# BadgerTechnologies/navigation

Hardware: AMD Instinct MI355X
Metric: scored trajectories/sec (whole node) + costmap inflation cells/sec, 400x400 map (higher is better)
Workload: dtype f64

## Files before the change

### navigation_amd/csrc/costmap_kernels.hip

```cpp
#include "navgpu_device.h"

namespace navgpu {

__global__ void k_fill_u8(uint8_t* dst, uint8_t v, size_t n) {
  size_t i = (size_t)blockIdx.x * blockDim.x + threadIdx.x;
  size_t stride = (size_t)gridDim.x * blockDim.x;
  uint32_t w = v * 0x01010101u;
  uint4 q = make_uint4(w, w, w, w);
  size_t n16 = n / 16;
  for (size_t k = i; k < n16; k += stride) reinterpret_cast<uint4*>(dst)[k] = q;
  for (size_t k = n16 * 16 + i; k < n; k += stride) dst[k] = v;
}
__global__ void k_fill_u32(uint32_t* dst, uint32_t v, size_t n) {
  size_t i = (size_t)blockIdx.x * blockDim.x + threadIdx.x;
  size_t stride = (size_t)gridDim.x * blockDim.x;
  for (size_t k = i; k < n; k += stride) dst[k] = v;
}
void launch_fill_u8(uint8_t* dst, uint8_t v, size_t n, hipStream_t s) {
  if (!n) return;
  size_t blocks = (n / 16 + 255) / 256;
  if (blocks < 1) blocks = 1;
  if (blocks > 4096) blocks = 4096;
  hipLaunchKernelGGL(k_fill_u8, dim3((unsigned)blocks), dim3(256), 0, s, dst, v, n);
}
void launch_fill_u32(uint32_t* dst, uint32_t v, size_t n, hipStream_t s) {
  if (!n) return;
  size_t blocks = (n + 255) / 256;
  if (blocks > 4096) blocks = 4096;
  hipLaunchKernelGGL(k_fill_u32, dim3((unsigned)blocks), dim3(256), 0, s, dst, v, n);
}

__global__ void k_static_interpret(uint8_t* dst, const int8_t* occ, uint32_t cells, uint32_t cells_padded, uint32_t count,
                                   int track_unknown_space, int trinary, int lethal_threshold, int unknown_cost_value) {
  uint32_t i = blockIdx.x * blockDim.x + threadIdx.x;
  if (i >= cells) return;
  uint8_t value = (uint8_t)occ[i];
  uint8_t lethal_thr = (uint8_t)lethal_threshold;
  uint8_t unknown = (uint8_t)unknown_cost_value;
  uint8_t out;
  if (track_unknown_space && value == unknown)
    out = kNoInfo;
  else if (!track_unknown_space && value == unknown)
    out = kFree;
  else if (value >= lethal_thr)
    out = kLethal;
  else if (trinary)
    out = kFree;
  else {
    double scale = (double)value / lethal_thr;
    out = (uint8_t)(scale * kLethal);
  }
  for (uint32_t k = 0; k < count; ++k) dst[(size_t)k * cells_padded + i] = out;
}
void launch_static_interpret(uint8_t* dst, const int8_t* occ, uint32_t cells, uint32_t cells_padded, uint32_t count,
                             int track_unknown_space, int trinary, int lethal_threshold, int unknown_cost_value, hipStream_t s) {
  hipLaunchKernelGGL(k_static_interpret, dim3((cells + 255) / 256), dim3(256), 0, s, dst, occ, cells, cells_padded, count,
                     track_unknown_space, trinary, lethal_threshold, unknown_cost_value);
}

__global__ void k_export_window(const uint8_t* master, uint32_t nx, uint32_t x0, uint32_t y0, uint32_t w, uint32_t h, int8_t* out) {
  const uint32_t i = blockIdx.x * blockDim.x + threadIdx.x;
  if (i >= w * h) return;
  const uint32_t y = i / w, x = i - y * w;
  const uint32_t v = master[(size_t)(y0 + y) * nx + x0 + x];
  int8_t o;
  if (v == 0) o = 0;
  else if (v == 253) o = 99;
  else if (v == 254) o = 100;
  else if (v == 255) o = -1;
  else o = (int8_t)(1 + (97 * ((int)v - 1)) / 251);
  out[i] = o;
}
void launch_export_window(const uint8_t* master, uint32_t nx, uint32_t x0, uint32_t y0, uint32_t w, uint32_t h, int8_t* out, hipStream_t s) {
  hipLaunchKernelGGL(k_export_window, dim3((w * h + 255) / 256), dim3(256), 0, s, master, nx, x0, y0, w, h, out);
}

template <class T>
__global__ __launch_bounds__(256) void k_shift(const T* src, T* dst, CostmapDev cm, uint32_t first, T fill) {
  const uint32_t inst = first + blockIdx.y;
  const int ox = cm.shift[2 * inst], oy = cm.shift[2 * inst + 1];
  const T* s = src + (size_t)inst * cm.cells_padded;
  T* d = dst + (size_t)inst * cm.cells_padded;
  for (uint32_t i = blockIdx.x * blockDim.x + threadIdx.x; i < cm.cells; i += gridDim.x * blockDim.x) {
    const int y = i / cm.nx, x = i - y * cm.nx;
    const int sx = x + ox, sy = y + oy;
    d[i] = (sx >= 0 && sy >= 0 && sx < (int)cm.nx && sy < (int)cm.ny) ? s[sy * cm.nx + sx] : fill;
  }
}
void launch_shift_u8(const uint8_t* src, uint8_t* dst, const CostmapDev& cm, uint32_t first, uint32_t count, uint8_t fill, hipStream_t s) {
  dim3 grid(min((cm.cells + 255) / 256, 64u), count);
  hipLaunchKernelGGL(k_shift<uint8_t>, grid, dim3(256), 0, s, src, dst, cm, first, fill);
}
void launch_shift_u32(const uint32_t* src, uint32_t* dst, const CostmapDev& cm, uint32_t first, uint32_t count, uint32_t fill, hipStream_t s) {
  dim3 grid(min((cm.cells + 255) / 256, 64u), count);
  hipLaunchKernelGGL(k_shift<uint32_t>, grid, dim3(256), 0, s, src, dst, cm, first, fill);
}

template <class F>
__device__ __forceinline__ void raytrace3d(uint32_t nx, double x0, double y0, double z0, double x1, double y1, double z1,
                                           uint32_t max_length, F&& at) {
  int dx = int(x1) - int(x0), dy = int(y1) - int(y0), dz = int(z1) - int(z0);
  uint32_t abs_dx = dx < 0 ? -dx : dx, abs_dy = dy < 0 ? -dy : dy, abs_dz = dz < 0 ? -dz : dz;
  int offset_dx = dx > 0 ? 1 : -1;
  int offset_dy = (dy > 0 ? 1 : -1) * (int)nx;
  int offset_dz = dz > 0 ? 1 : -1;
  uint32_t z_mask = ((1u << 16) | 1u) << (uint32_t)z0;
  uint32_t offset = (uint32_t)y0 * nx + (uint32_t)x0;
  double dist = sqrt((x0 - x1) * (x0 - x1) + (y0 - y1) * (y0 - y1) + (z0 - z1) * (z0 - z1));
  double scale = fmin(1.0, (double)max_length / dist);
  uint32_t abs_da, abs_db, abs_dc;
  int off_a, off_b, off_c, role_a, role_b, role_c;
  uint32_t mmax = abs_dy > abs_dz ? abs_dy : abs_dz;
  if (abs_dx >= mmax) {
    abs_da = abs_dx; abs_db = abs_dy; abs_dc = abs_dz;
    off_a = offset_dx; off_b = offset_dy; off_c = offset_dz;
    role_a = 0; role_b = 0; role_c = 1;
  } else if (abs_dy >= abs_dz) {
    abs_da = abs_dy; abs_db = abs_dx; abs_dc = abs_dz;
    off_a = offset_dy; off_b = offset_dx; off_c = offset_dz;
    role_a = 0; role_b = 0; role_c = 1;
  } else {
    abs_da = abs_dz; abs_db = abs_dx; abs_dc = abs_dy;
    off_a = offset_dz; off_b = offset_dx; off_c = offset_dy;
    role_a = 1; role_b = 0; role_c = 0;
  }
  auto step = [&](int role, int v) {
    if (role == 0)
      offset += v;
    else {
      if (v > 0)
        z_mask <<= 1;
      else
        z_mask >>= 1;
    }
  };
  uint32_t lim = (uint32_t)(scale * abs_da);
  uint32_t end = lim < abs_da ? lim : abs_da;
  int error_b = abs_da / 2, error_c = abs_da / 2;
  for (uint32_t i = 0; i < end; ++i) {
    at(offset, z_mask);
    step(role_a, off_a);
    error_b += abs_db;
    error_c += abs_dc;
    if ((uint32_t)error_b >= abs_da) {
      step(role_b, off_b);
      error_b -= abs_da;
    }
    if ((uint32_t)error_c >= abs_da) {
      step(role_c, off_c);
      error_c -= abs_da;
    }
  }
  at(offset, z_mask);
// ... 275 lines not shown
  b.store(st->bounds);
  int x0, xn, y0, yn;
  enforceBounds(g, b.min_x, b.min_y, x0, y0);
  enforceBounds(g, b.max_x, b.max_y, xn, yn);
  x0 = x0 > 0 ? x0 : 0;
  xn = ((int)g.nx < xn + 1) ? (int)g.nx : xn + 1;
  y0 = y0 > 0 ? y0 : 0;
  yn = ((int)g.ny < yn + 1) ? (int)g.ny : yn + 1;
  st->box[0] = x0;
  st->box[1] = xn;
  st->box[2] = y0;
  st->box[3] = yn;
  st->box_valid = !(xn < x0 || yn < y0);
  return st->box_valid;
}

__device__ __forceinline__ void clearFootprintPolygon(const CostmapDev& cm, const Geom& g, uint32_t inst, uint8_t* layer, uint32_t tid,
                                                      uint32_t* s_vx, uint32_t* s_vy, uint32_t* colmin, uint32_t* colmax, int* s_poly_ok) {
  const uint32_t nfp = cm.fp_n[inst];
  if (tid == 0) *s_poly_ok = nfp >= 3;
  __syncthreads();
  if (tid < nfp) {
    uint32_t mx, my;
    bool ok = worldToMap(g, cm.fp_world[((size_t)inst * kMaxFootprint + tid) * 2], cm.fp_world[((size_t)inst * kMaxFootprint + tid) * 2 + 1], mx, my);
    s_vx[tid] = mx;
    s_vy[tid] = my;
    if (!ok) atomicAnd(s_poly_ok, 0);
  }
  __syncthreads();
  if (!*s_poly_ok) return;
  uint32_t minx = 0xFFFFFFFFu, maxx = 0;
  for (uint32_t i = 0; i < nfp; ++i) {
    minx = s_vx[i] < minx ? s_vx[i] : minx;
    maxx = s_vx[i] > maxx ? s_vx[i] : maxx;
  }
  const uint32_t span = maxx - minx + 1;
  if (span > 1024) return;
  for (uint32_t c = tid; c < span; c += blockDim.x) {
    colmin[c] = 0xFFFFFFFFu;
    colmax[c] = 0;
  }
  __syncthreads();
  if (tid < nfp) {
    uint32_t e1 = (tid + 1 == nfp) ? 0 : tid + 1;
    raytrace2d(g.nx, s_vx[tid], s_vy[tid], s_vx[e1], s_vy[e1], 0xFFFFFFFFu, [&](uint32_t off) {
      uint32_t y = off / g.nx, x = off - y * g.nx;
      atomicMin(&colmin[x - minx], y);
      atomicMax(&colmax[x - minx], y);
    });
  }
  __syncthreads();
  for (uint32_t c = tid >> 4; c < span; c += blockDim.x >> 4) {
    uint32_t lo = colmin[c], hi = colmax[c];
    if (lo == 0xFFFFFFFFu) continue;
    for (uint32_t y = lo + (tid & 15); y <= hi; y += 16) layer[y * g.nx + minx + c] = kFree;
  }
}

template <bool VOXEL>
__global__ __launch_bounds__(256) void k_obstacle(CostmapDev cm, uint32_t first, const double* bounds_io_in, double* bounds_io_out,
                                                  int only_bounds) {
  const uint32_t inst = first + blockIdx.x, tid = threadIdx.x;
  ObstacleGrids L;
  L.g = Geom{cm.origin[2 * inst], cm.origin[2 * inst + 1], cm.res, cm.nx, cm.ny};
  L.layer = cm.obst + (size_t)inst * cm.cells_padded;
  L.vox = VOXEL ? cm.voxel + (size_t)inst * cm.cells_padded : nullptr;
  L.size_z = VOXEL ? (uint32_t)(cm.z_voxels > 16 ? 16 : cm.z_voxels) : 0;
  L.unknown_thr = VOXEL ? (uint32_t)(cm.unknown_threshold + (16 - cm.z_voxels)) : 0;
  L.mark_thr = VOXEL ? (uint32_t)cm.mark_threshold : 0;
  InstCostmapState* st = cm.state + inst;
  __shared__ double red[4][4];
  __shared__ int s_box_valid;
  __shared__ uint32_t colmin[1024], colmax[1024];
  __shared__ uint32_t s_vx[kMaxFootprint], s_vy[kMaxFootprint];
  __shared__ int s_poly_ok;

  const bool has_obs_layer = (cm.layers & (NAVGPU_LAYER_OBSTACLE | NAVGPU_LAYER_VOXEL)) && cm.obs_enabled;
  BoundsAcc b{1e30, 1e30, -1e30, -1e30};
  if (tid == 0) boundsSeed(cm, L.g, st, bounds_io_in, only_bounds, has_obs_layer, b);

  if (has_obs_layer) {
    const uint32_t ob = inst * cm.max_obs, oe = ob + cm.obs_count[inst];
    const float* inst_points = cm.points + (size_t)inst * cm.max_points * 3;
    for (int pass = 0; pass < (VOXEL ? 2 : 1); ++pass) {
      for (uint32_t o = ob; o < oe; ++o) {
        const ObsCsr obs = cm.obs[o];
        if (!(obs.flags & NAVGPU_OBS_CLEARING)) continue;
        if (!VOXEL)
          clearRays2D(L, obs, inst_points + (size_t)obs.first_point * 3, tid, b);
        else
          clearRaysVoxel(cm, L, obs, inst_points + (size_t)obs.first_point * 3, pass, tid, b);
      }
      __syncthreads();
    }
    if (VOXEL && L.mark_thr > 0)
      markPointsOrdered(cm, L, ob, oe, inst_points, cm.mark_seq + (size_t)inst * cm.max_points, tid, b);
    else
      for (uint32_t o = ob; o < oe; ++o) {
        const ObsCsr obs = cm.obs[o];
        if (!(obs.flags & NAVGPU_OBS_MARKING)) continue;
        markPoints<VOXEL>(cm, L, obs, inst_points + (size_t)obs.first_point * 3, tid, b);
      }
    footprintTouch(cm, inst, tid, b);
  }

  reduceBounds(b, red, tid);
  if (tid == 0) s_box_valid = finishBounds(cm, L.g, st, b, bounds_io_out, only_bounds);
  __syncthreads();
  if (has_obs_layer && cm.footprint_clearing && s_box_valid)
    clearFootprintPolygon(cm, L.g, inst, L.layer, tid, s_vx, s_vy, colmin, colmax, &s_poly_ok);
}

__global__ __launch_bounds__(256) void k_reset_bounding_box(CostmapDev cm, uint32_t first, const double* boxes_world) {
  const uint32_t inst = first + blockIdx.x;
  const Geom g{cm.origin[2 * inst], cm.origin[2 * inst + 1], cm.res, cm.nx, cm.ny};
  const double* bw = boxes_world + 4 * blockIdx.x;
  int x0, y0, xn, yn;
  enforceBounds(g, bw[0], bw[1], x0, y0);
  enforceBounds(g, bw[2], bw[3], xn, yn);
  uint8_t* layer = cm.obst + (size_t)inst * cm.cells_padded;
  if (xn > x0 && yn > y0) {
    const uint32_t w = (uint32_t)(xn - x0), n = w * (uint32_t)(yn - y0);
    for (uint32_t i = threadIdx.x; i < n; i += blockDim.x) layer[(uint32_t)(y0 + i / w) * g.nx + (uint32_t)x0 + i % w] = cm.obstacle_default;
  }
  if (threadIdx.x == 0) {
    InstCostmapState* st = cm.state + inst;
    if (!st->has_extra_bounds) {
      st->extra[0] = st->extra[1] = 1e6;
      st->extra[2] = st->extra[3] = -1e6;
    }
    st->extra[0] = (bw[0] < st->extra[0]) ? bw[0] : st->extra[0];
    st->extra[1] = (bw[1] < st->extra[1]) ? bw[1] : st->extra[1];
    st->extra[2] = (st->extra[2] < bw[2]) ? bw[2] : st->extra[2];
    st->extra[3] = (st->extra[3] < bw[3]) ? bw[3] : st->extra[3];
    st->has_extra_bounds = 1;
  }
}
__global__ __launch_bounds__(256) void k_reset_window(uint8_t* grid, size_t stride, uint32_t nx, uint32_t x0, uint32_t y0, uint32_t xn, uint32_t yn, uint8_t value) {
  uint8_t* gp = grid + (size_t)blockIdx.x * stride;
  const uint32_t w = xn - x0, n = w * (yn - y0);
  for (uint32_t i = threadIdx.x; i < n; i += blockDim.x) gp[(y0 + i / w) * nx + x0 + i % w] = value;
}
void launch_reset_window(uint8_t* grid, size_t stride, uint32_t count, uint32_t nx, uint32_t x0, uint32_t y0, uint32_t xn, uint32_t yn, uint8_t value, hipStream_t s) {
  hipLaunchKernelGGL(k_reset_window, dim3(count), dim3(256), 0, s, grid, stride, nx, x0, y0, xn, yn, value);
}
void launch_reset_bounding_box(const CostmapDev& cm, uint32_t first, uint32_t count, const double* boxes_world, hipStream_t s) {
  hipLaunchKernelGGL(k_reset_bounding_box, dim3(count), dim3(256), 0, s, cm, first, boxes_world);
}

struct UpdateBox {
  int x0, y0, xn, yn;
};
__device__ __forceinline__ bool updateBox(const CostmapDev& cm, const int32_t* boxes, uint32_t k, uint32_t inst, UpdateBox& box) {
  if (boxes) {
    box = UpdateBox{boxes[4 * k + 0], boxes[4 * k + 1], boxes[4 * k + 2], boxes[4 * k + 3]};
    return true;
  }
  const InstCostmapState* st = cm.state + inst;
  if (!st->box_valid) return false;
  box.x0 = st->box[0];
  box.xn = st->box[1];
  box.y0 = st->box[2];
  box.yn = st->box[3];
  return true;
}
__device__ __forceinline__ UpdateBox inflateBox(const UpdateBox& box, int R, uint32_t nx, uint32_t ny) {
  return UpdateBox{max(0, box.x0 - R), max(0, box.y0 - R), min((int)nx, box.xn + R), min((int)ny, box.yn + R)};
}

void launch_obstacle(const CostmapDev& cm, uint32_t first, uint32_t count, const double* bounds_in, int only_bounds, hipStream_t s) {
  double* bounds_out = const_cast<double*>(bounds_in);
  if (cm.layers & NAVGPU_LAYER_VOXEL)
    hipLaunchKernelGGL(k_obstacle<true>, dim3(count), dim3(256), 0, s, cm, first, bounds_in, bounds_out, only_bounds);
  else
    hipLaunchKernelGGL(k_obstacle<false>, dim3(count), dim3(256), 0, s, cm, first, bounds_in, bounds_out, only_bounds);
}

__global__ __launch_bounds__(256) void k_merge(CostmapDev cm, uint32_t first, const int32_t* boxes, int static_received, int layer_only) {
  const uint32_t inst = first + blockIdx.y;
  UpdateBox box;
  if (!updateBox(cm, boxes, blockIdx.y, inst, box)) return;
  const int x0 = box.x0, y0 = box.y0, xn = box.xn, yn = box.yn;
  const uint32_t q = blockIdx.x * blockDim.x + threadIdx.x;
  const uint32_t base = q * 16;
  if (base >= cm.cells) return;
  const int row_first = base / cm.nx, row_last = (min(base + 15, cm.cells - 1)) / cm.nx;
  if (row_last < y0 || row_first >= yn) return;
  bool inside = false;
  if (row_first == row_last) {
    const int gx = base - row_first * cm.nx;
    if (gx + 15 < x0 || gx >= xn) return;
    inside = gx >= x0 && gx + 15 < xn && base + 15 < cm.cells && !layer_only;
  }
  const size_t off = (size_t)inst * cm.cells_padded + base;
  uint4 mv = make_uint4(0, 0, 0, 0);
  if (!inside) mv = *reinterpret_cast<const uint4*>(cm.master + off);
  const bool has_static = (cm.layers & NAVGPU_LAYER_STATIC) && static_received && !layer_only && !cm.stat_roll && cm.stat;
  const bool roll_static = cm.stat_roll != nullptr && !layer_only;
  double tfm[8] = {1, 0, 0, 0, 0, 1, 0, 0};
  double m_ox = 0, m_oy = 0;
  if (roll_static) {
    const double* T = cm.stat_tf + (size_t)inst * 12;
    tfm[0] = T[0]; tfm[1] = T[1]; tfm[2] = T[2]; tfm[3] = T[9];
    tfm[4] = T[3]; tfm[5] = T[4]; tfm[6] = T[5]; tfm[7] = T[10];
    m_ox = cm.origin[2 * inst];
    m_oy = cm.origin[2 * inst + 1];
  }
  const bool has_obst = (cm.layers & (NAVGPU_LAYER_OBSTACLE | NAVGPU_LAYER_VOXEL)) && cm.obs_enabled;
  uint4 sv = has_static ? *reinterpret_cast<const uint4*>(cm.stat + off) : make_uint4(0, 0, 0, 0);
  uint4 lv = has_obst ? *reinterpret_cast<const uint4*>(cm.obst + off) : make_uint4(0, 0, 0, 0);
  uint32_t mw[4] = {mv.x, mv.y, mv.z, mv.w}, sw[4] = {sv.x, sv.y, sv.z, sv.w}, lw[4] = {lv.x, lv.y, lv.z, lv.w};
  int y = row_first;
  int x = base - row_first * cm.nx;
  bool changed = false;
#pragma unroll
  for (int k = 0; k < 16; ++k) {
    if (base + k < cm.cells && x >= x0 && x < xn && y >= y0 && y < yn) {
      const int sh = (k & 3) * 8;
      uint8_t m = layer_only ? (uint8_t)((mw[k >> 2] >> sh) & 0xFF) : cm.master_default;
      if (has_static) {
        uint8_t sc = (sw[k >> 2] >> sh) & 0xFF;
        if (!cm.static_use_maximum)
          m = sc;
        else if (sc != kNoInfo && (m == kNoInfo || m < sc))
          m = sc;
      }
      if (roll_static) {
        const double wx = m_ox + (x + 0.5) * cm.res, wy = m_oy + (y + 0.5) * cm.res;
        const double px = tfm[0] * wx + tfm[1] * wy + tfm[2] * 0.0 + tfm[3];
        const double py = tfm[4] * wx + tfm[5] * wy + tfm[6] * 0.0 + tfm[7];
        if (!(px < cm.stat_ox || py < cm.stat_oy)) {
          const uint32_t smx = (uint32_t)(int)((px - cm.stat_ox) / cm.stat_res), smy = (uint32_t)(int)((py - cm.stat_oy) / cm.stat_res);
          if (smx < cm.stat_nx && smy < cm.stat_ny) {
            const uint8_t sc = cm.stat_roll[(size_t)smy * cm.stat_nx + smx];
            m = cm.static_use_maximum ? (sc > m ? sc : m) : sc;
          }
        }
      }
      if (has_obst) {
        uint8_t lc = (lw[k >> 2] >> sh) & 0xFF;
        if (lc != kNoInfo) {
          if (cm.combination_method == 0)
            m = lc;
          else if (cm.combination_method == 1 && (m == kNoInfo || m < lc))
            m = lc;
        }
      }
      mw[k >> 2] = (mw[k >> 2] & ~(0xFFu << sh)) | ((uint32_t)m << sh);
      changed = true;
    }
    if (++x == (int)cm.nx) {
      x = 0;
      ++y;
    }
  }
  if (changed) *reinterpret_cast<uint4*>(cm.master + off) = make_uint4(mw[0], mw[1], mw[2], mw[3]);
}

void launch_merge(const CostmapDev& cm, uint32_t first, uint32_t count, const int32_t* boxes, hipStream_t s, bool layer_only) {
  uint32_t groups = (cm.cells + 15) / 16;
  dim3 grid((groups + 255) / 256, count);
  hipLaunchKernelGGL(k_merge, grid, dim3(256), 0, s, cm, first, boxes, cm.static_received, layer_only ? 1 : 0);
}

constexpr int kTile = 64;
__global__ __launch_bounds__(256) void k_inflate(CostmapDev cm, uint32_t first, const int32_t* boxes) {
  extern __shared__ __align__(16) uint8_t lds[];
  const uint32_t inst = first + blockIdx.z;
  const int R = (int)cm.R;
  UpdateBox box;
  if (!updateBox(cm, boxes, blockIdx.z, inst, box)) return;
  box = inflateBox(box, R, cm.nx, cm.ny);
  const int min_i = box.x0, min_j = box.y0, max_i = box.xn, max_j = box.yn;
  const int tx0 = blockIdx.x * kTile, ty0 = blockIdx.y * kTile;
  if (tx0 - R >= max_i || tx0 + kTile + R <= min_i || ty0 - R >= max_j || ty0 + kTile + R <= min_j) return;

  const int W = kTile + 2 * R;
  const int WS = (W + 3) & ~3;
  uint8_t* seed = lds;
  uint8_t* hd = seed + W * WS;
  uint8_t* lut = hd + W * kTile;
  __shared__ int s_any;
  const uint32_t tid = threadIdx.x;
  uint8_t* master = cm.master + (size_t)inst * cm.cells_padded;
  if (tid == 0) s_any = 0;
  for (int i = tid; i < (R + 2) * (R + 2); i += blockDim.x) lut[i] = cm.lut[i];
  __syncthreads();
  int any = 0;
  for (int i = tid; i < W * W; i += blockDim.x) {
    int ly = i / W, lx = i - ly * W;
    int gx = tx0 - R + lx, gy = ty0 - R + ly;
    uint8_t f = 0;
    if (gx >= min_i && gx < max_i && gy >= min_j && gy < max_j) f = master[gy * cm.nx + gx] == kLethal;
    seed[ly * WS + lx] = f;
    any |= f;
  }
  if (any) s_any = 1;
  __syncthreads();
  if (!s_any) return;
  for (int i = tid; i < W * kTile; i += blockDim.x) {
    int ly = i / kTile, c = i - ly * kTile;
    const uint8_t* row = seed + ly * WS + c + R;
    uint8_t best = 255;
    for (int d = 0; d <= R; ++d) {
      if (row[d] | row[-d]) {
        best = (uint8_t)d;
        break;
      }
    }
    hd[i] = best;
  }
  __syncthreads();
  const int n = R + 2;
  for (int i = tid; i < kTile * kTile; i += blockDim.x) {
    int ry = i / kTile, c = i - ry * kTile;
    int gx = tx0 + c, gy = ty0 + ry;
    if (gx >= (int)cm.nx || gy >= (int)cm.ny) continue;
    uint8_t cost = 0;
    for (int dy = -R; dy <= R; ++dy) {
      uint8_t h = hd[(ry + R + dy) * kTile + c];
      if (h != 255) {
        int ady = dy < 0 ? -dy : dy;
        uint8_t cc = lut[h * n + ady];
        cost = cc > cost ? cc : cost;
      }
    }
    if (cost == 0) continue;
    uint8_t old = master[gy * cm.nx + gx];
    uint8_t nv = (old == kNoInfo && cost >= kInscribed) ? cost : (old > cost ? old : cost);
    if (nv != old) master[gy * cm.nx + gx] = nv;
  }
}

constexpr int kBX = 64, kBY = 32;
template <int RT>
__global__ __launch_bounds__(256) void k_inflate_bits(CostmapDev cm, uint32_t first, uint32_t count, const int32_t* boxes) {
  const uint32_t tbx = blockIdx.x >> 3, tby = blockIdx.y, rz = blockIdx.z * 8u + (blockIdx.x & 7u);
  if (rz >= count) return;
  const uint32_t inst = first + rz;
  const int R = RT > 0 ? RT : (int)cm.R;
  UpdateBox box;
  if (!updateBox(cm, boxes, rz, inst, box)) return;
  box = inflateBox(box, R, cm.nx, cm.ny);
  const int min_i = box.x0, min_j = box.y0, max_i = box.xn, max_j = box.yn;
  const int tx0 = (int)tbx * kBX, ty0 = (int)tby * kBY;
  if (tx0 - R >= max_i || tx0 + kBX + R <= min_i || ty0 - R >= max_j || ty0 + kBY + R <= min_j) return;

  constexpr int kMaxHR = kBY + 2 * 14;
  constexpr int kOct = (kMaxHR + 7) / 8;
  __shared__ uint32_t s_rows[kMaxHR][4];
  __shared__ uint32_t s_hd[kOct + 1][kBX];
  __shared__ uint8_t s_lut2[256];
  __shared__ int s_any;
  __shared__ uint32_t s_rowany[2];
  const uint32_t tid = threadIdx.x, lane = tid & 63, wave = tid >> 6;
  const int HR = kBY + 2 * R;
  uint8_t* master = cm.master + (size_t)inst * cm.cells_padded;
  if (tid == 0) s_any = 0;
  if (tid < 2) s_rowany[tid] = 0;
  s_lut2[tid] = cm.lut2[tid];
  __syncthreads();
  int any = 0;
  uint32_t rows_lo = 0, rows_hi = 0;
  constexpr int kSeedIt = (kMaxHR + 3) / 4;
  uint8_t cell[kSeedIt][2];
  const int gxa = tx0 - 32 + (int)lane, gxb = gxa + 64;
  const int lo_x = max(min_i, tx0 - R), lo_y = max(min_j, ty0 - R);
  const int hi_x = max(lo_x, min(max_i, tx0 + kBX + R) - 1), hi_y = max(lo_y, min(max_j, ty0 + kBY + R) - 1);
  const int cxa = min(min(max(gxa, lo_x), hi_x), (int)cm.nx - 1), cxb = min(min(max(gxb, lo_x), hi_x), (int)cm.nx - 1);
  const bool xa_ok = gxa >= min_i && gxa < max_i && gxa >= tx0 - R && gxa < tx0 + kBX + R;
  const bool xb_ok = gxb >= min_i && gxb < max_i && gxb >= tx0 - R && gxb < tx0 + kBX + R;
#pragma unroll
  for (int it = 0; it < kSeedIt; ++it) {
    const int gy = ty0 - R + (int)wave + 4 * it;
    const int cy = min(min(max(gy, lo_y), hi_y), (int)cm.ny - 1);
    cell[it][0] = master[cy * cm.nx + cxa];
    cell[it][1] = master[cy * cm.nx + cxb];
  }
#pragma unroll
  for (int it = 0; it < kSeedIt; ++it) {
    const int r = (int)wave + 4 * it, gy = ty0 - R + r;
    if (r < HR) {
      const bool row_ok = gy >= min_j && gy < max_j;
#pragma unroll
      for (int half = 0; half < 2; ++half) {
        const unsigned long long m = __ballot(row_ok && (half ? xb_ok : xa_ok) && cell[it][half] == kLethal);
        if (lane == 0) {
          s_rows[r][2 * half] = (uint32_t)m;
          s_rows[r][2 * half + 1] = (uint32_t)(m >> 32);
        }
        any |= m != 0ull;
        if (m != 0ull) {
          if (r < 32)
            rows_lo |= 1u << r;
          else
            rows_hi |= 1u << (r - 32);
        }
      }
    }
  }
  if (any && lane == 0) {
    s_any = 1;
    if (rows_lo) atomicOr(&s_rowany[0], rows_lo);
    if (rows_hi) atomicOr(&s_rowany[1], rows_hi);
  }
  __syncthreads();
  if (!s_any) return;
  const uint32_t lowmask = (1u << R) - 1u;
  for (int o = wave; o * 8 < HR; o += 4) {
    uint32_t packed = 0;
#pragma unroll
    for (int k = 0; k < 8; ++k) {
      const int r = o * 8 + k;
      uint32_t h = 15;
      if (r < HR && (s_rows[r][0] | s_rows[r][1] | s_rows[r][2] | s_rows[r][3]) != 0u) {
        const uint32_t sft = 32u + lane - (uint32_t)R;
        const uint32_t wi = sft >> 5, bs = sft & 31u;
        const unsigned long long two = ((unsigned long long)s_rows[r][wi + 1 < 4 ? wi + 1 : 3] << 32) | s_rows[r][wi];
        const uint32_t q = (uint32_t)(two >> bs);
        const uint32_t qr = q >> R;
        const uint32_t ql = q & lowmask;
        uint32_t dr = 15, dl = 15;
        if (qr & ((2u << R) - 1u)) dr = (uint32_t)__builtin_ctz(qr & ((2u << R) - 1u));
        if (ql) dl = (uint32_t)R - (31u - (uint32_t)__builtin_clz(ql));
        h = dr < dl ? dr : dl;
      }
      packed |= h << (4 * k);
    }
    s_hd[o][lane] = packed;
  }
  __syncthreads();
  uint32_t hw[5];
#pragma unroll
  for (int k = 0; k < 5; ++k) hw[k] = (wave + k) * 8 < (uint32_t)HR ? s_hd[wave + k][lane] : 0xFFFFFFFFu;
  if (__ballot((hw[0] & hw[1] & hw[2] & hw[3] & hw[4]) != 0xFFFFFFFFu) == 0ull) return;
  const int gx = tx0 + (int)lane;
  const int R2 = R * R;
  uint32_t bestr[8] = {0xFFFFu, 0xFFFFu, 0xFFFFu, 0xFFFFu, 0xFFFFu, 0xFFFFu, 0xFFFFu, 0xFFFFu};
  if (RT > 0) {
    const unsigned long long rowany = (((unsigned long long)s_rowany[1] << 32) | s_rowany[0]) >> (8u * wave);
    const uint32_t ra_lo = __builtin_amdgcn_readfirstlane((uint32_t)rowany), ra_hi = __builtin_amdgcn_readfirstlane((uint32_t)(rowany >> 32));
#pragma unroll
    for (int p = 0; p < 8 + 2 * RT; ++p) {
      if (((p < 32 ? ra_lo >> (p & 31) : ra_hi >> (p & 31)) & 1u) != 0u) {
        const uint32_t h = (hw[p >> 3] >> (4 * (p & 7))) & 15u;
        const uint32_t hh = h * h;
#pragma unroll
        for (int j = 0; j < 8; ++j) {
          const int dy = p - RT - j;
          if (dy >= -RT && dy <= RT) {
            const uint32_t d2 = hh + (uint32_t)(dy * dy);
            bestr[j] = d2 < bestr[j] ? d2 : bestr[j];
          }
        }
      }
    }
  }
#pragma unroll
  for (int j = 0; j < 8; ++j) {
    const int gy = ty0 + (int)wave * 8 + j;
    uint32_t best = bestr[j];
    if (RT == 0) {
      for (int dy = -R; dy <= R; ++dy) {
        const int p = j + R + dy;
        const uint32_t wsel = p >> 3;
        const uint32_t word = wsel == 0 ? hw[0] : (wsel == 1 ? hw[1] : (wsel == 2 ? hw[2] : (wsel == 3 ? hw[3] : hw[4])));
        const uint32_t h = (word >> (4 * (p & 7))) & 15u;
        const uint32_t d2 = h * h + (uint32_t)(dy * dy);
        best = d2 < best ? d2 : best;
      }
    }
    if (best > (uint32_t)R2 || gx >= (int)cm.nx || gy >= (int)cm.ny) continue;
    const uint8_t cost = s_lut2[best];
    if (cost == 0) continue;
    const uint8_t old = master[gy * cm.nx + gx];
    const uint8_t nv = (old == kNoInfo && cost >= kInscribed) ? cost : (old > cost ? old : cost);
    if (nv != old) master[gy * cm.nx + gx] = nv;
  }
}

constexpr uint32_t kPqSeenWords = 5120, kPqWinBytes = 65536;
constexpr size_t kPqLdsBytes = 150 * 1024;
constexpr uint32_t kPqTabEntries = 66 * 66;
__global__ __launch_bounds__(64) void k_inflate_pq(CostmapDev cm, uint32_t first, const int32_t* boxes) {
  extern __shared__ __align__(16) uint8_t pq_sm[];
  const uint32_t inst = first + blockIdx.x;
  const uint32_t tid = threadIdx.x;
  UpdateBox box;
  if (!updateBox(cm, boxes, blockIdx.x, inst, box)) return;
  uint8_t* master = cm.master + (size_t)inst * cm.cells_padded;
  uint8_t* seen_g = cm.pq_seen + (size_t)inst * cm.cells_padded;
  PqCell* heap_g = cm.pq_heap + (size_t)inst * cm.pq_cap;
  const uint32_t size_x = cm.nx, size_y = cm.ny;
  const int R = (int)cm.R;
  const uint32_t n = cm.R + 2;
  box = inflateBox(box, R, size_x, size_y);
  const int min_i = box.x0, min_j = box.y0, max_i = box.xn, max_j = box.yn;
  if (max_i <= min_i || max_j <= min_j) return;
  const int wx0 = max(0, min_i - R - 1), wy0 = max(0, min_j - R - 1), wx1 = min((int)size_x, max_i + R + 1), wy1 = min((int)size_y, max_j + R + 1);
  const uint32_t ww = (uint32_t)(wx1 - wx0), wh = (uint32_t)(wy1 - wy0), wcells = ww * wh;
  const bool seen_lds = wcells <= kPqSeenWords * 32u, win_lds = wcells <= kPqWinBytes;
  uint16_t* rank = reinterpret_cast<uint16_t*>(pq_sm);
  uint8_t* lut_l = pq_sm + kPqTabEntries * 2;
  const uint32_t seen_off = (kPqTabEntries * 3 + 15u) & ~15u;
  uint32_t* seen_l = reinterpret_cast<uint32_t*>(pq_sm + seen_off);
  const uint32_t win_off = seen_off + (seen_lds ? (((wcells + 31) / 32 * 4 + 15u) & ~15u) : 0u);
  uint8_t* win_l = pq_sm + win_off;
  const uint32_t heap_off = win_off + (win_lds ? ((wcells + 15u) & ~15u) : 0u);
  PqCell* heap_l = reinterpret_cast<PqCell*>(pq_sm + heap_off);
  const long heap_lds = (long)((kPqLdsBytes - heap_off) / sizeof(PqCell));
  for (uint32_t i = tid; i < n * n; i += 64) {
    rank[i] = reinterpret_cast<const uint16_t*>(cm.dist_lut)[i];
    lut_l[i] = cm.lut[i];
  }
  if (seen_lds) {
    for (uint32_t i = tid; i < (wcells + 31) / 32; i += 64) seen_l[i] = 0;
  } else {
    for (uint32_t i = tid * 16; i < cm.cells_padded; i += 64 * 16) *reinterpret_cast<uint4*>(seen_g + i) = make_uint4(0, 0, 0, 0);
  }
  if (win_lds)
    for (uint32_t i = tid; i < wcells; i += 64) {
      const uint32_t y = i / ww, x = i - y * ww;
      win_l[i] = master[(uint32_t)(wy0 + (int)y) * size_x + (uint32_t)(wx0 + (int)x)];
    }
  __syncthreads();
  if (tid == 0) {
    long len = 0;
    auto hget = [&](long i) -> PqCell { return i < heap_lds ? heap_l[i] : heap_g[i]; };
    auto hset = [&](long i, const PqCell& v) {
      if (i < heap_lds)
        heap_l[i] = v;
      else
        heap_g[i] = v;
    };
    auto widx = [&](uint32_t mx, uint32_t my) { return (my - (uint32_t)wy0) * ww + (mx - (uint32_t)wx0); };
    auto seenGet = [&](uint32_t index, uint32_t mx, uint32_t my) -> bool {
      if (seen_lds) {
        const uint32_t w = widx(mx, my);
        return (seen_l[w >> 5] >> (w & 31)) & 1u;
      }
      return seen_g[index] != 0;
    };
    auto seenSet = [&](uint32_t index, uint32_t mx, uint32_t my) {
      if (seen_lds) {
        const uint32_t w = widx(mx, my);
        seen_l[w >> 5] |= 1u << (w & 31);
      } else {
        seen_g[index] = 1;
      }
    };
    auto pushHeap = [&](long hole, const PqCell& value) {
      long parent = (hole - 1) / 2;
      while (hole > 0) {
        const PqCell pv = hget(parent);
        if (!(pv.rank > value.rank)) break;
        hset(hole, pv);
        hole = parent;
        parent = (hole - 1) / 2;
      }
      hset(hole, value);
    };
    auto probe = [&](bool in_map, uint32_t index, uint32_t mx, uint32_t my, uint32_t sx, uint32_t sy) -> uint32_t {
      if (!in_map) return 0xFFFFu;
      const uint32_t dx = mx > sx ? mx - sx : sx - mx, dy = my > sy ? my - sy : sy - my;
      const uint32_t r = rank[dx * n + dy];
      return seenGet(index, mx, my) ? 0xFFFFu : r;
    };
    auto push = [&](uint32_t r, uint32_t index, uint32_t mx, uint32_t my, uint32_t sx, uint32_t sy) {
      if (r == 0xFFFFu) return;
      if ((uint64_t)len >= cm.pq_cap) return;
      PqCell c;
      c.index = index;
      c.rank = (uint16_t)r;
      c.sdx = (int8_t)((int)sx - (int)mx);
      c.sdy = (int8_t)((int)sy - (int)my);
      pushHeap(len++, c);
    };
    auto enqueue = [&](uint32_t index, uint32_t mx, uint32_t my, uint32_t sx, uint32_t sy) { push(probe(true, index, mx, my, sx, sy), index, mx, my, sx, sy); };
    for (int j = min_j; j < max_j; j++)
      for (int i = min_i; i < max_i; i++) {
        const uint32_t index = (uint32_t)j * size_x + (uint32_t)i;
        const uint8_t c0 = win_lds ? win_l[widx((uint32_t)i, (uint32_t)j)] : master[index];
        if (c0 == kLethal) enqueue(index, i, j, i, j);
      }
    while (len > 0) {
      const PqCell cur = hget(0);
      if (len > 1) {
        const PqCell value = hget(len - 1);
        const long l = len - 1;
        long hole = 0, child = 0;
        while (child < (l - 1) / 2) {
          child = 2 * (child + 1);
          const PqCell a = hget(child), b = hget(child - 1);
          if (a.rank > b.rank) {
            child--;
            hset(hole, b);
          } else {
            hset(hole, a);
          }
          hole = child;
        }
        if ((l & 1) == 0 && child == (l - 2) / 2) {
          child = 2 * (child + 1);
          hset(hole, hget(child - 1));
          hole = child - 1;
        }
        pushHeap(hole, value);
      }
      --len;
      const uint32_t index = cur.index;
      const uint32_t my = index / size_x, mx = index - my * size_x;
      if (seenGet(index, mx, my)) continue;
      seenSet(index, mx, my);
      const uint32_t sx = (uint32_t)((int)mx + cur.sdx), sy = (uint32_t)((int)my + cur.sdy);
      const uint32_t dx = mx > sx ? mx - sx : sx - mx, dy = my > sy ? my - sy : sy - my;
      const uint8_t cost = lut_l[dx * n + dy];
      uint8_t* cellp = win_lds ? &win_l[widx(mx, my)] : &master[index];
      const uint8_t old_cost = *cellp;
      if (old_cost == kNoInfo && cost >= kInscribed)
        *cellp = cost;
      else
        *cellp = old_cost > cost ? old_cost : cost;
      const uint32_t r0 = probe(mx > 0, index - 1, mx - 1, my, sx, sy), r1 = probe(my > 0, index - size_x, mx, my - 1, sx, sy),
                     r2 = probe(mx < size_x - 1, index + 1, mx + 1, my, sx, sy), r3 = probe(my < size_y - 1, index + size_x, mx, my + 1, sx, sy);
      push(r0, index - 1, mx - 1, my, sx, sy);
      push(r1, index - size_x, mx, my - 1, sx, sy);
      push(r2, index + 1, mx + 1, my, sx, sy);
      push(r3, index + size_x, mx, my + 1, sx, sy);
    }
  }
  __syncthreads();
  if (win_lds)
    for (uint32_t i = tid; i < wcells; i += 64) {
      const uint32_t y = i / ww, x = i - y * ww;
      master[(uint32_t)(wy0 + (int)y) * size_x + (uint32_t)(wx0 + (int)x)] = win_l[i];
    }
}

void launch_inflate(const CostmapDev& cm, uint32_t first, uint32_t count, const int32_t* boxes, hipStream_t s) {
  if (!cm.infl_enabled) return;
  const int R = (int)cm.R;
  if (cm.infl_pq) {
    if (!cm.pq_heap || !cm.pq_seen || !cm.dist_lut) return;
    hipFuncSetAttribute((const void*)k_inflate_pq, hipFuncAttributeMaxDynamicSharedMemorySize, (int)kPqLdsBytes);
    hipLaunchKernelGGL(k_inflate_pq, dim3(count), dim3(64), kPqLdsBytes, s, cm, first, boxes);
    return;
  }
  if (cm.lut2_ok && R >= 1 && R <= 14) {
    dim3 grid(8u * ((cm.nx + kBX - 1) / kBX), (cm.ny + kBY - 1) / kBY, (count + 7u) / 8u);
    if (R == 11)
      hipLaunchKernelGGL(k_inflate_bits<11>, grid, dim3(256), 0, s, cm, first, count, boxes);
    else
      hipLaunchKernelGGL(k_inflate_bits<0>, grid, dim3(256), 0, s, cm, first, count, boxes);
    return;
  }
  const int W = kTile + 2 * R, WS = (W + 3) & ~3;
  size_t lds = (size_t)W * WS + (size_t)W * kTile + (size_t)(R + 2) * (R + 2);
  dim3 grid((cm.nx + kTile - 1) / kTile, (cm.ny + kTile - 1) / kTile, count);
  hipLaunchKernelGGL(k_inflate, grid, dim3(256), lds, s, cm, first, boxes);
}

}
```

Baseline: 6.370 billion.

## Vectorize costmap merge with SWAR word rules and streamline bit-inflation kernel

Result: faster. 6.606 billion (median of 6 runs) (+3.7%).

```diff
diff --git a/navigation_amd/csrc/costmap_kernels.hip b/navigation_amd/csrc/costmap_kernels.hip
--- a/navigation_amd/csrc/costmap_kernels.hip
+++ b/navigation_amd/csrc/costmap_kernels.hip
@@ -1,4 +1,5 @@
 #include "navgpu_device.h"
+#include "costmap_word_rules.h"
 
 namespace navgpu {
 
@@ -580,17 +581,14 @@
   int x0, y0, xn, yn;
 };
 __device__ __forceinline__ bool updateBox(const CostmapDev& cm, const int32_t* boxes, uint32_t k, uint32_t inst, UpdateBox& box) {
-  if (boxes) {
-    box = UpdateBox{boxes[4 * k + 0], boxes[4 * k + 1], boxes[4 * k + 2], boxes[4 * k + 3]};
-    return true;
-  }
   const InstCostmapState* st = cm.state + inst;
-  if (!st->box_valid) return false;
-  box.x0 = st->box[0];
-  box.xn = st->box[1];
-  box.y0 = st->box[2];
-  box.yn = st->box[3];
-  return true;
+  const int32_t* p = boxes ? boxes + 4 * (size_t)k : st->box;
+  const int b0 = p[0], b1 = p[1], b2 = p[2], b3 = p[3];
+  box.x0 = b0;
+  box.y0 = boxes ? b1 : b2;
+  box.xn = boxes ? b2 : b1;
+  box.yn = b3;
+  return boxes ? true : st->box_valid != 0;
 }
 __device__ __forceinline__ UpdateBox inflateBox(const UpdateBox& box, int R, uint32_t nx, uint32_t ny) {
   return UpdateBox{max(0, box.x0 - R), max(0, box.y0 - R), min((int)nx, box.xn + R), min((int)ny, box.yn + R)};
@@ -604,7 +602,53 @@
     hipLaunchKernelGGL(k_obstacle<false>, dim3(count), dim3(256), 0, s, cm, first, bounds_in, bounds_out, only_bounds);
 }
 
-__global__ __launch_bounds__(256) void k_merge(CostmapDev cm, uint32_t first, const int32_t* boxes, int static_received, int layer_only) {
+template <bool ALIGNED, int STATIC, int OBST, bool LAYER_ONLY>
+__global__ __launch_bounds__(256) void k_merge(CostmapDev cm, uint32_t first, const int32_t* boxes, word_rules::FastDiv div_nx,
+                                                     word_rules::FastDiv div_gpr) {
+  using namespace word_rules;
+  const uint32_t inst = first + blockIdx.y;
+  UpdateBox box;
+  if (!updateBox(cm, boxes, blockIdx.y, inst, box)) return;
+  const int x0 = box.x0, y0 = box.y0, xn = box.xn, yn = box.yn;
+  const uint32_t wq = blockIdx.x * 256u + (__builtin_amdgcn_readfirstlane(threadIdx.x) & ~63u);
+  if (wq * 16u >= cm.cells) return;
+  const int wrow_first = (int)fastDiv(wq * 16u, div_nx), wrow_last = (int)fastDiv(min(wq * 16u + 1023u, cm.cells - 1u), div_nx);
+  if (wrow_last < y0 || wrow_first >= yn) return;
+  const uint32_t q = blockIdx.x * 256u + threadIdx.x;
+  const uint32_t base = q * 16u;
+  if (base >= cm.cells) return;
+  uint32_t bits;
+  if (ALIGNED) {
+    const uint32_t gpr = cm.nx >> 4, row = fastDiv(q, div_gpr);
+    bits = ((int)row >= y0 && (int)row < yn) ? boxBits((int)((q - row * gpr) << 4), x0, xn) : 0u;
+  } else {
+    int y = (int)fastDiv(base, div_nx);
+    int x = (int)(base - (uint32_t)y * cm.nx);
+    bits = 0;
+#pragma unroll
+    for (int k = 0; k < 16; ++k) {
+      if (base + k < cm.cells && x >= x0 && x < xn && y >= y0 && y < yn) bits |= 1u << k;
+      if (++x == (int)cm.nx) {
+        x = 0;
+        ++y;
+      }
+    }
+  }
+  if (bits == 0u) return;
+  const size_t off = (size_t)inst * cm.cells_padded + base;
+  const uint4 sv = STATIC ? *reinterpret_cast<const uint4*>(cm.stat + off) : make_uint4(0, 0, 0, 0);
+  const uint4 lv = OBST ? *reinterpret_cast<const uint4*>(cm.obst + off) : make_uint4(0, 0, 0, 0);
+  uint4 mv = make_uint4(0, 0, 0, 0);
+  if (LAYER_ONLY || bits != 0xFFFFu) mv = *reinterpret_cast<const uint4*>(cm.master + off);
+  uint4 out;
+  out.x = mergeWord<STATIC, OBST, LAYER_ONLY>(mv.x, sv.x, lv.x, boxBytes(bits, 0), cm.master_default);
+  out.y = mergeWord<STATIC, OBST, LAYER_ONLY>(mv.y, sv.y, lv.y, boxBytes(bits, 1), cm.master_default);
+  out.z = mergeWord<STATIC, OBST, LAYER_ONLY>(mv.z, sv.z, lv.z, boxBytes(bits, 2), cm.master_default);
+  out.w = mergeWord<STATIC, OBST, LAYER_ONLY>(mv.w, sv.w, lv.w, boxBytes(bits, 3), cm.master_default);
+  *reinterpret_cast<uint4*>(cm.master + off) = out;
+}
+
+__global__ __launch_bounds__(256) void k_merge_bytes(CostmapDev cm, uint32_t first, const int32_t* boxes, int static_received, int layer_only) {
   const uint32_t inst = first + blockIdx.y;
   UpdateBox box;
   if (!updateBox(cm, boxes, blockIdx.y, inst, box)) return;
@@ -685,10 +729,51 @@
   if (changed) *reinterpret_cast<uint4*>(cm.master + off) = make_uint4(mw[0], mw[1], mw[2], mw[3]);
 }
 
+template <bool ALIGNED, int STATIC, int OBST, bool LAYER_ONLY>
+static void launchMergeWords(const CostmapDev& cm, uint32_t first, const int32_t* boxes, dim3 grid, hipStream_t s) {
+  hipLaunchKernelGGL((k_merge<ALIGNED, STATIC, OBST, LAYER_ONLY>), grid, dim3(256), 0, s, cm, first, boxes, word_rules::fastDivOf(cm.nx),
+                     word_rules::fastDivOf(cm.nx >= 16 ? cm.nx >> 4 : 1));
+}
+template <bool ALIGNED, int STATIC>
+static void launchMergeObst(const CostmapDev& cm, uint32_t first, const int32_t* boxes, dim3 grid, hipStream_t s, int obst, bool layer_only) {
+  if (layer_only) {
+    if (STATIC != 0) return;
+    switch (obst) {
+      case 0: return launchMergeWords<ALIGNED, 0, 0, true>(cm, first, boxes, grid, s);
+      case 1: return launchMergeWords<ALIGNED, 0, 1, true>(cm, first, boxes, grid, s);
+      default: return launchMergeWords<ALIGNED, 0, 2, true>(cm, first, boxes, grid, s);
+    }
+  }
+  switch (obst) {
+    case 0: return launchMergeWords<ALIGNED, STATIC, 0, false>(cm, first, boxes, grid, s);
+    case 1: return launchMergeWords<ALIGNED, STATIC, 1, false>(cm, first, boxes, grid, s);
+    default: return launchMergeWords<ALIGNED, STATIC, 2, false>(cm, first, boxes, grid, s);
+  }
+}
+template <bool ALIGNED>
+static void launchMergeStatic(const CostmapDev& cm, uint32_t first, const int32_t* boxes, dim3 grid, hipStream_t s, int stat, int obst, bool layer_only) {
+  switch (stat) {
+    case 0: return launchMergeObst<ALIGNED, 0>(cm, first, boxes, grid, s, obst, layer_only);
+    case 1: return launchMergeObst<ALIGNED, 1>(cm, first, boxes, grid, s, obst, layer_only);
+    default: return launchMergeObst<ALIGNED, 2>(cm, first, boxes, grid, s, obst, layer_only);
+  }
+}
+
 void launch_merge(const CostmapDev& cm, uint32_t first, uint32_t count, const int32_t* boxes, hipStream_t s, bool layer_only) {
   uint32_t groups = (cm.cells + 15) / 16;
   dim3 grid((groups + 255) / 256, count);
-  hipLaunchKernelGGL(k_merge, grid, dim3(256), 0, s, cm, first, boxes, cm.static_received, layer_only ? 1 : 0);
+  if ((cm.stat_roll != nullptr && !layer_only) || cm.cells >= 0x80000000u) {
+    hipLaunchKernelGGL(k_merge_bytes, grid, dim3(256), 0, s, cm, first, boxes, cm.static_received, layer_only ? 1 : 0);
+    return;
+  }
+  const bool has_static = (cm.layers & NAVGPU_LAYER_STATIC) && cm.static_received && !layer_only && cm.stat;
+  const bool has_obst = (cm.layers & (NAVGPU_LAYER_OBSTACLE | NAVGPU_LAYER_VOXEL)) && cm.obs_enabled;
+  const int stat = !has_static ? 0 : (cm.static_use_maximum ? 2 : 1);
+  const int obst = !has_obst ? 0 : (cm.combination_method == 0 ? 1 : (cm.combination_method == 1 ? 2 : 0));
+  if (cm.nx % 16 == 0)
+    launchMergeStatic<true>(cm, first, boxes, grid, s, stat, obst, layer_only);
+  else
+    launchMergeStatic<false>(cm, first, boxes, grid, s, stat, obst, layer_only);
 }
 
 constexpr int kTile = 64;
@@ -761,43 +846,42 @@
 }
 
 constexpr int kBX = 64, kBY = 32;
-template <int RT>
+template <int RT, bool BOXES>
 __global__ __launch_bounds__(256) void k_inflate_bits(CostmapDev cm, uint32_t first, uint32_t count, const int32_t* boxes) {
   const uint32_t tbx = blockIdx.x >> 3, tby = blockIdx.y, rz = blockIdx.z * 8u + (blockIdx.x & 7u);
   if (rz >= count) return;
   const uint32_t inst = first + rz;
   const int R = RT > 0 ? RT : (int)cm.R;
   UpdateBox box;
-  if (!updateBox(cm, boxes, rz, inst, box)) return;
+  if (BOXES) {
+    box = UpdateBox{boxes[4 * rz + 0], boxes[4 * rz + 1], boxes[4 * rz + 2], boxes[4 * rz + 3]};
+  } else {
+    const InstCostmapState* st = cm.state + inst;
+    box = UpdateBox{st->box[0], st->box[2], st->box[1], st->box[3]};
+    if (!st->box_valid) return;
+  }
+  const int tx0 = (int)tbx * kBX, ty0 = (int)tby * kBY;
+  if (tx0 - 2 * R >= box.xn || tx0 + kBX + 2 * R <= box.x0 || ty0 - 2 * R >= box.yn || ty0 + kBY + 2 * R <= box.y0) return;
   box = inflateBox(box, R, cm.nx, cm.ny);
   const int min_i = box.x0, min_j = box.y0, max_i = box.xn, max_j = box.yn;
-  const int tx0 = (int)tbx * kBX, ty0 = (int)tby * kBY;
-  if (tx0 - R >= max_i || tx0 + kBX + R <= min_i || ty0 - R >= max_j || ty0 + kBY + R <= min_j) return;
 
   constexpr int kMaxHR = kBY + 2 * 14;
   constexpr int kOct = (kMaxHR + 7) / 8;
-  __shared__ uint32_t s_rows[kMaxHR][4];
+  __shared__ __align__(16) uint32_t s_rows[kMaxHR][4];
   __shared__ uint32_t s_hd[kOct + 1][kBX];
   __shared__ uint8_t s_lut2[256];
-  __shared__ int s_any;
-  __shared__ uint32_t s_rowany[2];
-  const uint32_t tid = threadIdx.x, lane = tid & 63, wave = tid >> 6;
+  const uint32_t tid = threadIdx.x, lane = tid & 63, wave = (__builtin_amdgcn_readfirstlane(tid) >> 6) & 3u;
   const int HR = kBY + 2 * R;
   uint8_t* master = cm.master + (size_t)inst * cm.cells_padded;
-  if (tid == 0) s_any = 0;
-  if (tid < 2) s_rowany[tid] = 0;
   s_lut2[tid] = cm.lut2[tid];
-  __syncthreads();
-  int any = 0;
-  uint32_t rows_lo = 0, rows_hi = 0;
-  constexpr int kSeedIt = (kMaxHR + 3) / 4;
+  constexpr int kSeedIt = ((RT > 0 ? kBY + 2 * RT : kMaxHR) + 3) / 4;
   uint8_t cell[kSeedIt][2];
   const int gxa = tx0 - 32 + (int)lane, gxb = gxa + 64;
   const int lo_x = max(min_i, tx0 - R), lo_y = max(min_j, ty0 - R);
   const int hi_x = max(lo_x, min(max_i, tx0 + kBX + R) - 1), hi_y = max(lo_y, min(max_j, ty0 + kBY + R) - 1);
   const int cxa = min(min(max(gxa, lo_x), hi_x), (int)cm.nx - 1), cxb = min(min(max(gxb, lo_x), hi_x), (int)cm.nx - 1);
-  const bool xa_ok = gxa >= min_i && gxa < max_i && gxa >= tx0 - R && gxa < tx0 + kBX + R;
-  const bool xb_ok = gxb >= min_i && gxb < max_i && gxb >= tx0 - R && gxb < tx0 + kBX + R;
+  const unsigned long long xa_ok = __builtin_amdgcn_ballot_w64(gxa >= min_i && gxa < max_i && gxa >= tx0 - R && gxa < tx0 + kBX + R);
+  const unsigned long long xb_ok = __builtin_amdgcn_ballot_w64(gxb >= min_i && gxb < max_i && gxb >= tx0 - R && gxb < tx0 + kBX + R);
 #pragma unroll
   for (int it = 0; it < kSeedIt; ++it) {
     const int gy = ty0 - R + (int)wave + 4 * it;
@@ -807,55 +891,45 @@
   }
 #pragma unroll
   for (int it = 0; it < kSeedIt; ++it) {
-    const int r = (int)wave + 4 * it, gy = ty0 - R + r;
+    const int r = (int)wave + 4 * it;
     if (r < HR) {
-      const bool row_ok = gy >= min_j && gy < max_j;
+      const unsigned long long ma = __builtin_amdgcn_ballot_w64(cell[it][0] == kLethal) & xa_ok;
+      const unsigned long long mb = __builtin_amdgcn_ballot_w64(cell[it][1] == kLethal) & xb_ok;
+      *reinterpret_cast<uint4*>(s_rows[r]) = make_uint4((uint32_t)ma, (uint32_t)(ma >> 32), (uint32_t)mb, (uint32_t)(mb >> 32));
+    }
+  }
+  __syncthreads();
+  unsigned long long rowany_tile;
+  {
+    const uint4 w = *reinterpret_cast<const uint4*>(s_rows[lane < (uint32_t)HR ? lane : 0u]);
+    const int gyl = ty0 - R + (int)lane;
+    rowany_tile = __builtin_amdgcn_ballot_w64(lane < (uint32_t)HR && gyl >= min_j && gyl < max_j && (w.x | w.y | w.z | w.w) != 0u);
+  }
+  if (rowany_tile == 0ull) return;
+  const uint32_t lowmask = (1u << R) - 1u;
+  const uint32_t sft = 32u + lane - (uint32_t)R;
+  const uint32_t wi = sft >> 5, bs = sft & 31u;
+  for (int o = wave; o * 8 < HR; o += 4) {
+    const uint32_t oct = (uint32_t)(rowany_tile >> (8 * o)) & 0xFFu;
+    uint32_t near = 0;
+    if (oct != 0u) {
 #pragma unroll
-      for (int half = 0; half < 2; ++half) {
-        const unsigned long long m = __ballot(row_ok && (half ? xb_ok : xa_ok) && cell[it][half] == kLethal);
-        if (lane == 0) {
-          s_rows[r][2 * half] = (uint32_t)m;
-          s_rows[r][2 * half + 1] = (uint32_t)(m >> 32);
+      for (int k = 0; k < 8; ++k) {
+        if ((oct >> k) & 1u) {
+          const int r = o * 8 + k;
+          const unsigned long long two = ((unsigned long long)s_rows[r][wi + 1] << 32) | s_rows[r][wi];
+          const uint32_t q = (uint32_t)(two >> bs);
+          const uint32_t qr = q >> R;
+          const uint32_t ql = q & lowmask;
+          uint32_t dr = 15, dl = 15;
+          if (qr & ((2u << R) - 1u)) dr = (uint32_t)__builtin_ctz(qr & ((2u << R) - 1u));
+          if (ql) dl = (uint32_t)R - (31u - (uint32_t)__builtin_clz(ql));
+          const uint32_t h = dr < dl ? dr : dl;
+          near |= (15u - h) << (4 * k);
         }
-        any |= m != 0ull;
-        if (m != 0ull) {
-          if (r < 32)
-            rows_lo |= 1u << r;
-          else
-            rows_hi |= 1u << (r - 32);
-        }
-      }
-    }
-  }
-  if (any && lane == 0) {
-    s_any = 1;
-    if (rows_lo) atomicOr(&s_rowany[0], rows_lo);
-    if (rows_hi) atomicOr(&s_rowany[1], rows_hi);
-  }
-  __syncthreads();
-  if (!s_any) return;
-  const uint32_t lowmask = (1u << R) - 1u;
-  for (int o = wave; o * 8 < HR; o += 4) {
-    uint32_t packed = 0;
-#pragma unroll
-    for (int k = 0; k < 8; ++k) {
-      const int r = o * 8 + k;
-      uint32_t h = 15;
-      if (r < HR && (s_rows[r][0] | s_rows[r][1] | s_rows[r][2] | s_rows[r][3]) != 0u) {
-        const uint32_t sft = 32u + lane - (uint32_t)R;
-        const uint32_t wi = sft >> 5, bs = sft & 31u;
-        const unsigned long long two = ((unsigned long long)s_rows[r][wi + 1 < 4 ? wi + 1 : 3] << 32) | s_rows[r][wi];
-        const uint32_t q = (uint32_t)(two >> bs);
-        const uint32_t qr = q >> R;
-        const uint32_t ql = q & lowmask;
-        uint32_t dr = 15, dl = 15;
-        if (qr & ((2u << R) - 1u)) dr = (uint32_t)__builtin_ctz(qr & ((2u << R) - 1u));
-        if (ql) dl = (uint32_t)R - (31u - (uint32_t)__builtin_clz(ql));
-        h = dr < dl ? dr : dl;
-      }
-      packed |= h << (4 * k);
-    }
-    s_hd[o][lane] = packed;
+      }
+    }
+    s_hd[o][lane] = ~near;
   }
   __syncthreads();
   uint32_t hw[5];
@@ -864,26 +938,38 @@
   if (__ballot((hw[0] & hw[1] & hw[2] & hw[3] & hw[4]) != 0xFFFFFFFFu) == 0ull) return;
   const int gx = tx0 + (int)lane;
   const int R2 = R * R;
-  uint32_t bestr[8] = {0xFFFFu, 0xFFFFu, 0xFFFFu, 0xFFFFu, 0xFFFFu, 0xFFFFu, 0xFFFFu, 0xFFFFu};
+  uint8_t oldb[8];
+  {
+    const int cgx = min(gx, (int)cm.nx - 1);
+#pragma unroll
+    for (int j = 0; j < 8; ++j) oldb[j] = master[min(ty0 + (int)wave * 8 + j, (int)cm.ny - 1) * cm.nx + cgx];
+  }
+  typedef unsigned short u16x2 __attribute__((ext_vector_type(2)));
+  constexpr unsigned short kFar = 0x7000;
+  u16x2 bestp[4] = {{0xFFFFu, 0xFFFFu}, {0xFFFFu, 0xFFFFu}, {0xFFFFu, 0xFFFFu}, {0xFFFFu, 0xFFFFu}};
   if (RT > 0) {
-    const unsigned long long rowany = (((unsigned long long)s_rowany[1] << 32) | s_rowany[0]) >> (8u * wave);
-    const uint32_t ra_lo = __builtin_amdgcn_readfirstlane((uint32_t)rowany), ra_hi = __builtin_amdgcn_readfirstlane((uint32_t)(rowany >> 32));
+    const unsigned long long rowany = rowany_tile >> (8u * wave);
+    const uint32_t ra_lo = (uint32_t)rowany, ra_hi = (uint32_t)(rowany >> 32);
 #pragma unroll
     for (int p = 0; p < 8 + 2 * RT; ++p) {
       if (((p < 32 ? ra_lo >> (p & 31) : ra_hi >> (p & 31)) & 1u) != 0u) {
         const uint32_t h = (hw[p >> 3] >> (4 * (p & 7))) & 15u;
-        const uint32_t hh = h * h;
+        const uint32_t hh2 = (h * 0x10001u) * h;
 #pragma unroll
-        for (int j = 0; j < 8; ++j) {
-          const int dy = p - RT - j;
-          if (dy >= -RT && dy <= RT) {
-            const uint32_t d2 = hh + (uint32_t)(dy * dy);
-            bestr[j] = d2 < bestr[j] ? d2 : bestr[j];
+        for (int i = 0; i < 4; ++i) {
+          const int dy0 = p - RT - 2 * i, dy1 = dy0 - 1;
+          const bool in0 = dy0 >= -RT && dy0 <= RT, in1 = dy1 >= -RT && dy1 <= RT;
+          if (in0 || in1) {
+            const uint32_t dd = (in0 ? (uint32_t)(dy0 * dy0) : kFar) | ((in1 ? (uint32_t)(dy1 * dy1) : kFar) << 16);
+            bestp[i] = __builtin_elementwise_min(bestp[i], __builtin_bit_cast(u16x2, hh2 + dd));
           }
         }
       }
     }
   }
+  uint32_t bestr[8];
+#pragma unroll
+  for (int j = 0; j < 8; ++j) bestr[j] = (j & 1) ? bestp[j >> 1].y : bestp[j >> 1].x;
 #pragma unroll
   for (int j = 0; j < 8; ++j) {
     const int gy = ty0 + (int)wave * 8 + j;
@@ -898,12 +984,11 @@
         best = d2 < best ? d2 : best;
       }
     }
-    if (best > (uint32_t)R2 || gx >= (int)cm.nx || gy >= (int)cm.ny) continue;
-    const uint8_t cost = s_lut2[best];
-    if (cost == 0) continue;
-    const uint8_t old = master[gy * cm.nx + gx];
+    const uint8_t cost = s_lut2[best < 255u ? best : 255u];
+    const uint8_t old = oldb[j];
     const uint8_t nv = (old == kNoInfo && cost >= kInscribed) ? cost : (old > cost ? old : cost);
-    if (nv != old) master[gy * cm.nx + gx] = nv;
+    const uint32_t write = (uint32_t)(best <= (uint32_t)R2) & (uint32_t)(gx < (int)cm.nx) & (uint32_t)(gy < (int)cm.ny) & (uint32_t)(nv != old);
+    if (write) master[gy * cm.nx + gx] = nv;
   }
 }
 
@@ -1077,9 +1162,9 @@
   if (cm.lut2_ok && R >= 1 && R <= 14) {
     dim3 grid(8u * ((cm.nx + kBX - 1) / kBX), (cm.ny + kBY - 1) / kBY, (count + 7u) / 8u);
     if (R == 11)
-      hipLaunchKernelGGL(k_inflate_bits<11>, grid, dim3(256), 0, s, cm, first, count, boxes);
+      hipLaunchKernelGGL((boxes ? k_inflate_bits<11, true> : k_inflate_bits<11, false>), grid, dim3(256), 0, s, cm, first, count, boxes);
     else
-      hipLaunchKernelGGL(k_inflate_bits<0>, grid, dim3(256), 0, s, cm, first, count, boxes);
+      hipLaunchKernelGGL((boxes ? k_inflate_bits<0, true> : k_inflate_bits<0, false>), grid, dim3(256), 0, s, cm, first, count, boxes);
     return;
   }
   const int W = kTile + 2 * R, WS = (W + 3) & ~3;
diff --git a/navigation_amd/csrc/costmap_word_rules.h b/navigation_amd/csrc/costmap_word_rules.h
--- /dev/null
+++ b/navigation_amd/csrc/costmap_word_rules.h
@@ -0,0 +1,73 @@
+#pragma once
+#include <stdint.h>
+
+#if defined(__HIPCC__) || defined(__CUDACC__)
+#define WORD_RULE __host__ __device__ __forceinline__
+#else
+#define WORD_RULE inline
+#endif
+
+namespace word_rules {
+
+constexpr uint32_t kTop = 0x80808080u, kLow7 = 0x7F7F7F7Fu;
+
+WORD_RULE uint32_t isNoInformation(uint32_t w) { return ((w & kLow7) + 0x01010101u) & w & kTop; }
+
+WORD_RULE uint32_t isBelow(uint32_t a, uint32_t b) {
+  const uint32_t d = (a | kTop) - (b & kLow7);
+  return ((~a & b) | (~(a ^ b) & ~d)) & kTop;
+}
+
+WORD_RULE uint32_t maskOf(uint32_t flags) { return (flags << 1) - (flags >> 7); }
+
+WORD_RULE uint32_t choose(uint32_t mask, uint32_t a, uint32_t b) { return (a & mask) | (b & ~mask); }
+
+WORD_RULE uint32_t updateWithTrueOverwrite(uint32_t , uint32_t layer) { return layer; }
+
+WORD_RULE uint32_t updateWithOverwrite(uint32_t master, uint32_t layer) {
+  return choose(maskOf(~isNoInformation(layer) & kTop), layer, master);
+}
+
+WORD_RULE uint32_t updateWithMax(uint32_t master, uint32_t layer) {
+  const uint32_t take = ~isNoInformation(layer) & (isNoInformation(master) | isBelow(master, layer));
+  return choose(maskOf(take & kTop), layer, master);
+}
+
+WORD_RULE uint32_t boxBits(int gx, int x0, int xn) {
+  int lo = x0 - gx, hi = xn - gx;
+  lo = lo < 0 ? 0 : (lo > 16 ? 16 : lo);
+  hi = hi < 0 ? 0 : (hi > 16 ? 16 : hi);
+  return ((1u << hi) - 1u) & ~((1u << lo) - 1u);
+}
+
+WORD_RULE uint32_t boxBytes(uint32_t bits, int j) {
+  uint32_t m = (((bits >> (4 * j)) & 15u) * 0x00204081u) & 0x01010101u;
+  m |= m << 1;
+  m |= m << 2;
+  return m | (m << 4);
+}
+
+WORD_RULE uint32_t resetMap(uint8_t default_value) { return (uint32_t)default_value * 0x01010101u; }
+
+template <int STATIC, int OBST, bool LAYER_ONLY>
+WORD_RULE uint32_t mergeWord(uint32_t old, uint32_t stat, uint32_t obst, uint32_t in_box, uint8_t default_value) {
+  uint32_t m = LAYER_ONLY ? old : resetMap(default_value);
+  if (STATIC == 1) m = updateWithTrueOverwrite(m, stat);
+  if (STATIC == 2) m = updateWithMax(m, stat);
+  if (OBST == 1) m = updateWithOverwrite(m, obst);
+  if (OBST == 2) m = updateWithMax(m, obst);
+  return choose(in_box, m, old);
+}
+
+struct FastDiv {
+  uint32_t mul, shift;
+};
+inline FastDiv fastDivOf(uint32_t d) {
+  uint32_t l = 0;
+  while ((1ull << l) < d) ++l;
+  const uint64_t p = 1ull << (31 + l);
+  return FastDiv{(uint32_t)((p + d - 1) / d), 31 + l};
+}
+WORD_RULE uint32_t fastDiv(uint32_t n, FastDiv f) { return (uint32_t)(((uint64_t)n * f.mul) >> f.shift); }
+
+}
```
